# basilevh/tcow

Measured on AMD Instinct MI355X. Metric: train clips/sec (T=30, 240x320), higher is better.
Workload: dtype bf16; 1 GPU; TCOW Seeker train step: T=30 240x320 patch16, 12-layer divided space-time ViT (D=768), num_queries=3, causal_attention=1, 1 clip/GPU; clips_per_gpu=1, num_queries=3, parallelism=dp1, optimizer=AdamW lr 1e-4, clip 0.3

## Files before the change

### include/tcow_hip.h

```cpp
#ifndef TCOW_HIP_H
#define TCOW_HIP_H

#ifdef __cplusplus
extern "C" {
#endif

#define TCOW_OK 0
#define TCOW_ERR_INVALID_ARG (-1)
#define TCOW_ERR_LAUNCH (-2)
#define TCOW_ERR_UNSUPPORTED (-3)

#define TCOW_F32 0
#define TCOW_BF16 1
#define TCOW_F32X3 2

#define TCOW_ACT_NONE 0
#define TCOW_ACT_GELU 1
#define TCOW_ACT_DGELU 2
#define TCOW_ACT_GELU_DSAVE 3
#define TCOW_ACT_MUL_AUX 4

#define TCOW_ABI_VERSION 14
int tcow_version(void);
const char* tcow_last_error(void);
// ... 36 lines not shown
    float* bias_grad;
    int accumulate;
} tcow_tn_problem;
long tcow_gemm_tn_grouped_workspace_bytes(int dtype, int n, const tcow_tn_problem* problems);
int tcow_gemm_tn_grouped(void* stream, int dtype, int n, const tcow_tn_problem* problems, void* workspace, long workspace_bytes);
int tcow_gemm_tn_group_max(void);

typedef struct {
    int M, N, K;
    const float* A; long sai, sak;
    const float* B; long sbj, sbk;
    float* C; long ldc;
    int accumulate;
} tcow_sgemm;
int tcow_sgemm_x3_batched(void* stream, int n, const tcow_sgemm* problems);

int tcow_layernorm_fwd(void* stream, int dtype, int rows, int D, const float* x, long ldx, const float* gamma,
                       const float* beta, float eps, void* y, long ldy, float* mean, float* rstd);
long tcow_layernorm_bwd_workspace_bytes(int D);
int tcow_layernorm_bwd(void* stream, int dtype, int rows, int D, const void* dy, long lddy, const float* x, long ldx,
                       const float* mean, const float* rstd, const float* gamma, const float* dres, long lddres,
                       float* dx, long lddx, float* dgamma, float* dbeta, int accumulate, void* workspace,
                       long workspace_bytes, void* dx_cast, long lddx_cast, const float* cast_row_scale,
                       const float* colsum_row_scale, float* colsum_out);
typedef struct {
    const float* part; int parts, D;
    float* dgamma; float* dbeta; float* colsum_out;
    int accumulate;
} tcow_ln_fold_job;
int tcow_layernorm_bwd_parts(int rows, int with_colsum);
int tcow_layernorm_fold(void* stream, int n, const tcow_ln_fold_job* jobs);

typedef struct {
// ... 125 lines not shown
```

### tcow_amd/_lib.py

```python
import ctypes
import os

_HERE = os.path.dirname(os.path.abspath(__file__))
LIB_PATH = os.environ.get('TCOW_LIB') or os.path.join(_HERE, 'libtcow_hip.so')
LIB_PATH_FP16 = os.path.join(_HERE, 'libtcow_hip_fp16.so')

TCOW_F32, TCOW_BF16, TCOW_F32X3 = 0, 1, 2
ACT_NONE, ACT_GELU, ACT_DGELU, ACT_GELU_DSAVE, ACT_MUL_AUX = 0, 1, 2, 3, 4


class TcowError(RuntimeError):
    """Raised when a libtcow_hip entry point returns a non-zero status (message from tcow_last_error)."""


class AttnShape(ctypes.Structure):
    _fields_ = [('B', ctypes.c_int), ('T', ctypes.c_int), ('S', ctypes.c_int), ('D', ctypes.c_int),
                ('heads', ctypes.c_int), ('causal', ctypes.c_int), ('dtype', ctypes.c_int)]


class GemmArgs(ctypes.Structure):
    _fields_ = [('M', ctypes.c_int), ('N', ctypes.c_int), ('K', ctypes.c_int), ('dtype', ctypes.c_int),
                ('A', ctypes.c_void_p), ('lda', ctypes.c_long), ('W', ctypes.c_void_p), ('ldw', ctypes.c_long),
                ('C', ctypes.c_void_p), ('ldc', ctypes.c_long), ('out_f32', ctypes.c_int),
                ('bias', ctypes.c_void_p), ('row_scale', ctypes.c_void_p), ('resid', ctypes.c_void_p),
                ('ldr', ctypes.c_long), ('act', ctypes.c_int), ('aux', ctypes.c_void_p), ('ldaux', ctypes.c_long), ('tile', ctypes.c_int),
                ('bias2', ctypes.c_void_p), ('row_scale2', ctypes.c_void_p)]


class SGemm(ctypes.Structure):
    _fields_ = [('M', ctypes.c_int), ('N', ctypes.c_int), ('K', ctypes.c_int),
                ('A', ctypes.c_void_p), ('sai', ctypes.c_long), ('sak', ctypes.c_long),
                ('B', ctypes.c_void_p), ('sbj', ctypes.c_long), ('sbk', ctypes.c_long),
                ('C', ctypes.c_void_p), ('ldc', ctypes.c_long), ('accumulate', ctypes.c_int)]


class TnProblem(ctypes.Structure):
    _fields_ = [('M', ctypes.c_int), ('N', ctypes.c_int), ('K', ctypes.c_int),
                ('dY', ctypes.c_void_p), ('ldy', ctypes.c_long), ('X', ctypes.c_void_p), ('ldx', ctypes.c_long),
                ('dW', ctypes.c_void_p), ('lddw', ctypes.c_long), ('bias_grad', ctypes.c_void_p), ('accumulate', ctypes.c_int)]


class LnFoldJob(ctypes.Structure):
    _fields_ = [('part', ctypes.c_void_p), ('parts', ctypes.c_int), ('D', ctypes.c_int), ('dgamma', ctypes.c_void_p), ('dbeta', ctypes.c_void_p),
                ('colsum_out', ctypes.c_void_p), ('accumulate', ctypes.c_int)]


class MaskLossArgs(ctypes.Structure):
    _fields_ = [('n_frames', ctypes.c_long), ('frame_len', ctypes.c_long), ('frames_per_seq', ctypes.c_long),
# ... 14 lines not shown
    'tcow_version': (_i, []),
    'tcow_last_error': (ctypes.c_char_p, []),
    'tcow_gemm_nt': (_i, [_vp, ctypes.POINTER(GemmArgs)]),
    'tcow_gemm_nt_skinny_workspace_bytes': (_l, [_i, _i, _i]),
    'tcow_gemm_nt_skinny': (_i, [_vp, ctypes.POINTER(GemmArgs), _i, _vp, _l]),
    'tcow_prof_gemm_begin': (_i, [_i]),
    'tcow_prof_gemm_end': (_i, [ctypes.POINTER(ctypes.c_double), ctypes.POINTER(ctypes.c_double), ctypes.POINTER(ctypes.c_long)]),
    'tcow_prof_attn_begin': (_i, [_i]),
    'tcow_prof_attn_end': (_i, [_vp, _vp, _vp, _vp]),
    'tcow_gemm_tn_workspace_bytes': (_l, [_i, _i, _i]),
    'tcow_gemm_tn': (_i, [_vp, _i, _i, _i, _i, _vp, _l, _vp, _l, _vp, _l, _vp, _i, _vp, _l]),
    'tcow_gemm_tn_grouped_workspace_bytes': (_l, [_i, _i, _vp]),
    'tcow_gemm_tn_grouped': (_i, [_vp, _i, _i, _vp, _vp, _l]),
    'tcow_gemm_tn_group_max': (_i, []),
    'tcow_sgemm_x3_batched': (_i, [_vp, _i, _vp]),
    'tcow_layernorm_fwd': (_i, [_vp, _i, _i, _i, _vp, _l, _vp, _vp, _f, _vp, _l, _vp, _vp]),
    'tcow_layernorm_bwd_workspace_bytes': (_l, [_i]),
    'tcow_layernorm_bwd': (_i, [_vp, _i, _i, _i, _vp, _l, _vp, _l, _vp, _vp, _vp, _vp, _l, _vp, _l, _vp, _vp, _i, _vp, _l, _vp, _l, _vp, _vp, _vp]),
    'tcow_layernorm_bwd_parts': (_i, [_i, _i]),
    'tcow_layernorm_fold': (_i, [_vp, _i, _vp]),
    'tcow_attn_temporal_fwd': (_i, [_vp, _ash, _vp, _vp, _vp]),
    'tcow_attn_spatial_fwd': (_i, [_vp, _ash, _vp, _vp, _vp]),
    'tcow_attn_bwd_workspace_bytes': (_l, [_ash]),
    'tcow_attn_temporal_bwd': (_i, [_vp, _ash, _vp, _vp, _vp, _vp, _vp, _vp, _l]),
    'tcow_attn_spatial_bwd': (_i, [_vp, _ash, _vp, _vp, _vp, _vp, _vp, _vp, _l]),
    'tcow_attn_temporal_cached_fwd': (_i, [_vp, _ash, _i, _vp, _vp, _vp, _vp, _vp]),
    'tcow_cls_stream': (_i, [_vp, _i, _i, _i, _i, _vp, _vp, _vp]),
    'tcow_attn_temporal_pool_fwd': (_i, [_vp, _ash, _i, _i, _vp, _vp, _vp, _vp, _vp, _vp]),
    'tcow_cls_pool': (_i, [_vp, _i, _i, _i, _i, _vp, _vp, _i, _vp, _vp]),
    'tcow_attn_temporal_ragged_fwd': (_i, [_vp, _ash, _i, _i, _i, _vp, _vp, _vp, _vp, _vp, _vp, _vp, _vp, _vp]),
    'tcow_cls_ragged': (_i, [_vp, _i, _i, _i, _i, _vp, _vp, _i, _vp, _vp, _vp, _vp]),
# ... 76 lines not shown
```

### tcow_amd/csrc/gemm_x3.hip

```cpp
#include "gemm_f32.h"

namespace {

constexpr int XT = 128;
constexpr int XK = 32;
constexpr int XP = 80;
constexpr int XPLANE = XT * XP;

typedef __attribute__((ext_vector_type(8))) __bf16 x3_bf16x8;
typedef __attribute__((ext_vector_type(2))) __bf16 x3_bf16x2;
__device__ __forceinline__ uint32_t x3_pack(float a, float b) {
    f32x2 v = {a, b};
    return __builtin_bit_cast(uint32_t, __builtin_convertvector(v, x3_bf16x2));
}
__device__ __forceinline__ void split2(float x0, float x1, uint32_t& h, uint32_t& l) {
    h = x3_pack(x0, x1);
    l = x3_pack(x0 - __builtin_bit_cast(float, h << 16), x1 - __builtin_bit_cast(float, h & 0xffff0000u));
}

enum { LD_ANY = 0, LD_KVEC = 1, LD_RVEC = 2 };

template <int LD>
__device__ __forceinline__ void load_regs(const float* __restrict__ P, long s_row, long s_k, int row0, int nrows, int k0, int K, f32x4 (&v)[4], int tid) {
    if (LD == LD_KVEC) {
// ... 91 lines not shown
                uint32_t h, l;
                split2(v[e][2 * ps], v[e][2 * ps + 1], h, l);
                const int off = (iq + 32 * e) * XP + (kp + 8 * ps) * 4;
                *reinterpret_cast<uint32_t*>(hi_plane + off) = h;
                *reinterpret_cast<uint32_t*>(lo_plane + off) = l;
            }
    }
}

__device__ __forceinline__ int cdiv_dev(int a, int b) { return (a + b - 1) / b; }

__device__ __forceinline__ x3_bf16x8 frag(const char* plane, int row, int ks, int hi) {
    return __builtin_bit_cast(x3_bf16x8, *reinterpret_cast<const uint4*>(plane + row * XP + ks * 32 + hi * 16));
}

template <int LDA, int LDB>
__device__ __forceinline__ void gemm_x3_body(const F32Params& p, const int bid, const int kz, char* smem) {
    char* a_hi = smem; char* a_lo = smem + XPLANE; char* b_hi = smem + 2 * XPLANE; char* b_lo = smem + 3 * XPLANE;
    const int tid = threadIdx.x, lane = tid & 63, wave = tid >> 6;
    const int wm = wave >> 1, wn = wave & 1, l31 = lane & 31, hi = lane >> 5;
    const int tiles_n = cdiv_dev(p.N, XT), nblk = tiles_n * cdiv_dev(p.M, XT);
    const int q = nblk >> 3, rr = nblk & 7, xcd = bid & 7;
    const int pid = ((xcd < rr) ? xcd * (q + 1) : rr * (q + 1) + (xcd - rr) * q) + (bid >> 3);
    const int pm = pid / tiles_n;
    const int m0 = pm * XT, n0 = (pid - pm * tiles_n) * XT;
    const int kbeg = kz * p.kps;
    const int kend = (kbeg + p.kps < p.K) ? kbeg + p.kps : p.K;
    f32x16 acc[2][2];
#pragma unroll
    for (int i = 0; i < 2; ++i)
#pragma unroll
        for (int j = 0; j < 2; ++j)
// ... 24 lines not shown
                for (int j = 0; j < 2; ++j) {
                    acc[i][j] = __builtin_amdgcn_mfma_f32_32x32x16_bf16(bh[j], al[i], acc[i][j], 0, 0, 0);
                    acc[i][j] = __builtin_amdgcn_mfma_f32_32x32x16_bf16(bl[j], ah[i], acc[i][j], 0, 0, 0);
                    acc[i][j] = __builtin_amdgcn_mfma_f32_32x32x16_bf16(bh[j], ah[i], acc[i][j], 0, 0, 0);
                }
        }
        __syncthreads();
    };
    fetch(ra0, rb0, kbeg);
    __builtin_amdgcn_sched_barrier(0);
    fetch(ra1, rb1, kbeg + XK);
    __builtin_amdgcn_sched_barrier(0);
    for (int k0 = kbeg; k0 < kend; k0 += 2 * XK) {
        step(ra0, rb0, k0, k0 + 2 * XK);
        step(ra1, rb1, k0 + XK, k0 + 3 * XK);
    }
    constexpr int CT_LD = 68;
    float* ct = reinterpret_cast<float*>(smem) + wave * (32 * CT_LD);
    const int c4 = (lane & 15) * 4, r4 = lane >> 4;
    const int gn = n0 + wn * 64 + c4;
    const bool v16 = p.slab ? ((reinterpret_cast<uintptr_t>(p.slab) & 15) == 0 && (p.N & 3) == 0)
                            : (((reinterpret_cast<uintptr_t>(p.C) | reinterpret_cast<uintptr_t>(p.resid) | reinterpret_cast<uintptr_t>(p.aux) | reinterpret_cast<uintptr_t>(p.bias2)) & 15) == 0 &&
                               ((p.ldc | p.ldr | p.ldaux) & 3) == 0);
    float4 b4 = make_float4(0.f, 0.f, 0.f, 0.f);
    if (!p.slab && p.bias) {
        if (gn < p.N) b4.x = p.bias[gn];
        if (gn + 1 < p.N) b4.y = p.bias[gn + 1];
        if (gn + 2 < p.N) b4.z = p.bias[gn + 2];
        if (gn + 3 < p.N) b4.w = p.bias[gn + 3];
    }
// ... 21 lines not shown
                    if (slab) slab[(size_t)gm * p.N + gn + e] = xs[e];
                    else f32_epilogue_store(p, gm, gn + e, xs[e], bs[e]);
                }
            }
        }
    }
}

template <int LD>
__global__ __launch_bounds__(256, LD == LD_ANY ? 2 : 3) void gemm_x3_kernel(F32Params p) {
    __shared__ __attribute__((aligned(16))) char smem[4 * XPLANE];
    gemm_x3_body<LD, LD>(p, blockIdx.x, blockIdx.y, smem);
}

constexpr int X3_MAX_BATCH = 24;
struct X3Batch { F32Params p[X3_MAX_BATCH]; };
template <int LDA, int LDB>
__global__ __launch_bounds__(256, (LDA == LD_ANY || LDB == LD_ANY) ? 2 : 3) void gemm_x3_batch_kernel(X3Batch b) {
    __shared__ __attribute__((aligned(16))) char smem[4 * XPLANE];
    const F32Params& p = b.p[blockIdx.y];
    if ((int)blockIdx.x >= cdiv_dev(p.N, XT) * cdiv_dev(p.M, XT)) return;
    gemm_x3_body<LDA, LDB>(p, blockIdx.x, 0, smem);
}

}

int tcow_launch_slab_reduce(hipStream_t stream, const float* slab, int nz, long slab_stride, long rows, long cols, float* out, long ldo, int accumulate,
                            const float* bias_part, int bias_nparts, int bias_n, float* bias_out);

int tcow_gemm_nt_x3(hipStream_t stream, const tcow_gemm_args* a) {
    F32Params p;
    p.M = a->M; p.N = a->N; p.K = a->K;
    p.A = (const float*)a->A; p.sai = a->lda; p.sak = 1;
    p.B = (const float*)a->W; p.sbj = a->ldw; p.sbk = 1;
    p.C = a->C; p.ldc = a->ldc; p.bias = a->bias; p.row_scale = a->row_scale; p.resid = a->resid; p.ldr = a->ldr;
    p.act = a->act; p.aux = (float*)a->aux; p.ldaux = a->ldaux; p.bias2 = a->bias2; p.row_scale2 = a->row_scale2; p.kps = ((a->K + XK - 1) / XK) * XK; p.slab = nullptr;
    const bool vec = ((reinterpret_cast<uintptr_t>(p.A) | reinterpret_cast<uintptr_t>(p.B)) & 15) == 0 && ((p.sai | p.sbj | p.K) & 3) == 0;
// ... 27 lines not shown
    const bool vec = ((reinterpret_cast<uintptr_t>(dY) | reinterpret_cast<uintptr_t>(X)) & 15) == 0 && ((ldy | ldx | N | K) & 3) == 0;
    const dim3 grid(cdiv(K, XT) * cdiv(N, XT), nz);
    if (vec) hipLaunchKernelGGL(gemm_x3_kernel<LD_RVEC>, grid, dim3(256), 0, stream, p);
    else hipLaunchKernelGGL(gemm_x3_kernel<LD_ANY>, grid, dim3(256), 0, stream, p);
    TCOW_CHECK_LAUNCH();
    return tcow_launch_slab_reduce(stream, slab, nz, (long)N * K, N, K, dW, lddw, accumulate, bias_part, bias_nparts, N, bias_out);
}

static int x3_loader(const float* P, long s_row, long s_k, int nrows, int K) {
    const bool al = (reinterpret_cast<uintptr_t>(P) & 15) == 0;
    if (s_k == 1 && al && (s_row & 3) == 0 && (K & 3) == 0 && K >= 4) return LD_KVEC;
    if (s_row == 1 && al && (s_k & 3) == 0 && (nrows & 3) == 0 && nrows >= 4) return LD_RVEC;
    return LD_ANY;
}

extern "C" int tcow_sgemm_x3_batched(void* stream, int n, const tcow_sgemm* probs) {
    TCOW_CHECK_ARG(n >= 1 && n <= X3_MAX_BATCH && probs, "tcow_sgemm_x3_batched: 1 .. %d problems per call (got %d)", X3_MAX_BATCH, n);
    X3Batch b;
    int lda = -1, ldb = -1, maxtiles = 0;
    for (int i = 0; i < n; ++i) {
        const tcow_sgemm& s = probs[i];
        TCOW_CHECK_ARG(s.M > 0 && s.N > 0 && s.K > 0 && s.A && s.B && s.C && s.ldc >= s.N, "tcow_sgemm_x3_batched: bad problem %d", i);
        F32Params& p = b.p[i];
        p.M = s.M; p.N = s.N; p.K = s.K; p.A = s.A; p.sai = s.sai; p.sak = s.sak; p.B = s.B; p.sbj = s.sbj; p.sbk = s.sbk;
        p.C = s.C; p.ldc = s.ldc; p.bias = nullptr; p.row_scale = nullptr; p.resid = nullptr; p.ldr = 0; p.act = 0; p.aux = nullptr; p.ldaux = 0; p.bias2 = nullptr; p.row_scale2 = nullptr;
        p.kps = ((s.K + XK - 1) / XK) * XK; p.slab = nullptr;
        if (s.accumulate) { p.resid = s.C; p.ldr = s.ldc; }
        const int la = x3_loader(s.A, s.sai, s.sak, s.M, s.K), lb = x3_loader(s.B, s.sbj, s.sbk, s.N, s.K);
        lda = (lda < 0 || lda == la) ? la : LD_ANY; ldb = (ldb < 0 || ldb == lb) ? lb : LD_ANY;
        const int t = cdiv(s.N, XT) * cdiv(s.M, XT);
        if (t > maxtiles) maxtiles = t;
    }
    const dim3 grid(maxtiles, n);
    hipStream_t st = (hipStream_t)stream;
    if (lda == LD_KVEC && ldb == LD_KVEC) hipLaunchKernelGGL((gemm_x3_batch_kernel<LD_KVEC, LD_KVEC>), grid, dim3(256), 0, st, b);
    else if (lda == LD_KVEC && ldb == LD_RVEC) hipLaunchKernelGGL((gemm_x3_batch_kernel<LD_KVEC, LD_RVEC>), grid, dim3(256), 0, st, b);
    else if (lda == LD_RVEC && ldb == LD_RVEC) hipLaunchKernelGGL((gemm_x3_batch_kernel<LD_RVEC, LD_RVEC>), grid, dim3(256), 0, st, b);
    else if (lda == LD_RVEC && ldb == LD_ANY) hipLaunchKernelGGL((gemm_x3_batch_kernel<LD_RVEC, LD_ANY>), grid, dim3(256), 0, st, b);
    else hipLaunchKernelGGL((gemm_x3_batch_kernel<LD_ANY, LD_ANY>), grid, dim3(256), 0, st, b);
    TCOW_CHECK_LAUNCH();
    return TCOW_OK;
}
```

### tcow_amd/csrc/layernorm.hip

```cpp
#include <stdlib.h>

#include "common.h"

namespace {

constexpr int LN_MAXV = 8;

template <typename T, int NV, bool FULL>
__global__ __launch_bounds__(256) void ln_fwd_kernel(int rows, int D, const float* __restrict__ x, long ldx, const float* __restrict__ gamma,
                                                     const float* __restrict__ beta, float eps, T* __restrict__ y, long ldy,
                                                     float* __restrict__ mean_out, float* __restrict__ rstd_out) {
    const int lane = threadIdx.x & 63;
    const int nv = D >> 2;
    const int rstep = gridDim.x * 4;
    int row = blockIdx.x * 4 + (threadIdx.x >> 6);
    if (row >= rows) return;
    float4 g[NV], b[NV], nx[NV];
#pragma unroll
    for (int i = 0; i < NV; ++i) {
        const int c = lane + i * 64;
        if (FULL || c < nv) { g[i] = ld4(gamma + c * 4); b[i] = ld4(beta + c * 4); nx[i] = ld4(x + (size_t)row * ldx + c * 4); }
    }
    for (; row < rows; row += rstep) {
        float4 v[NV];
        float s = 0.f;
#pragma unroll
        for (int i = 0; i < NV; ++i) {
            const int c = lane + i * 64;
            if (FULL || c < nv) { v[i] = nx[i]; s += (v[i].x + v[i].y) + (v[i].z + v[i].w); }
        }
        if (row + rstep < rows) {
#pragma unroll
            for (int i = 0; i < NV; ++i) {
                const int c = lane + i * 64;
                if (FULL || c < nv) nx[i] = ld4(x + (size_t)(row + rstep) * ldx + c * 4);
            }
        }
        const float mean = wave_sum(s) / (float)D;
        float q = 0.f;
#pragma unroll
        for (int i = 0; i < NV; ++i) {
            const int c = lane + i * 64;
            if (FULL || c < nv) {
                const float a = v[i].x - mean, bb = v[i].y - mean, cc = v[i].z - mean, d = v[i].w - mean;
                q += (a * a + bb * bb) + (cc * cc + d * d);
            }
        }
        const float rstd = 1.0f / sqrtf(wave_sum(q) / (float)D + eps);
        if (lane == 0) {
            if (mean_out) mean_out[row] = mean;
// ... 120 lines not shown
        __syncthreads();
    }
}

}

int tcow_launch_row_reduce2(hipStream_t stream, const float* part, int nrows, long ld, int N1, float* out1, int N2, float* out2, int accumulate);
int tcow_launch_row_reduce_group(hipStream_t stream, int n, const float* const* part, const int* nrows, const long* ld, const int* N1, float* const* out1, const int* N2,
                                 float* const* out2, const int* N3, float* const* out3, const int* accumulate);
int tcow_launch_row_reduce3(hipStream_t stream, const float* part, int nrows, long ld, int N1, float* out1, int N2, float* out2, int N3, float* out3, int accumulate);

static const int kLnBwdBlocks = 768;
static const int kLnBwdBlocksCsum = 512;
static const int kLnFwdBlocks = 4096;

extern "C" {

int tcow_layernorm_fwd(void* stream, int dtype, int rows, int D, const float* x, long ldx, const float* gamma, const float* beta, float eps, void* y,
                       long ldy, float* mean, float* rstd) {
    TCOW_CHECK_ARG(rows > 0 && D > 0 && D % 4 == 0 && D <= 64 * 4 * LN_MAXV, "tcow_layernorm_fwd: D=%d must be a multiple of 4 and <= %d", D, 64 * 4 * LN_MAXV);
    TCOW_CHECK_ARG(x && gamma && beta && y && ldx % 4 == 0 && ldy % 4 == 0, "tcow_layernorm_fwd: bad pointers / strides");
    int fblocks = cdiv(rows, 4); if (fblocks > kLnFwdBlocks) fblocks = kLnFwdBlocks;
    const dim3 grid(fblocks), block(256);
    if (dtype != TCOW_BF16 && dtype != TCOW_F32) { tcow_set_error("tcow_layernorm_fwd: unknown dtype %d", dtype); return TCOW_ERR_INVALID_ARG; }
    const int nvl = (D / 4 + 63) / 64;
#define LN_FWD(NVV, FULLV)                                                                                                                               \
    do {                                                                                                                                          \
        if (dtype == TCOW_BF16) hipLaunchKernelGGL((ln_fwd_kernel<bf16_t, NVV, FULLV>), grid, block, 0, (hipStream_t)stream, rows, D, x, ldx, gamma, beta, eps, (bf16_t*)y, ldy, mean, rstd); \
        else hipLaunchKernelGGL((ln_fwd_kernel<float, NVV, FULLV>), grid, block, 0, (hipStream_t)stream, rows, D, x, ldx, gamma, beta, eps, (float*)y, ldy, mean, rstd); \
    } while (0)
    const bool full = D == 256 * nvl && nvl <= 4;
    if (full) { if (nvl == 1) LN_FWD(1, true); else if (nvl == 2) LN_FWD(2, true); else if (nvl == 3) LN_FWD(3, true); else LN_FWD(4, true); }
    else if (nvl <= 1) LN_FWD(1, false); else if (nvl == 2) LN_FWD(2, false); else if (nvl == 3) LN_FWD(3, false); else if (nvl == 4) LN_FWD(4, false); else LN_FWD(8, false);
#undef LN_FWD
    TCOW_CHECK_LAUNCH();
    return TCOW_OK;
}

long tcow_layernorm_bwd_workspace_bytes(int D) { return (long)kLnBwdBlocks * 3 * D * 4; }

int tcow_layernorm_bwd(void* stream, int dtype, int rows, int D, const void* dy, long lddy, const float* x, long ldx, const float* mean,
                       const float* rstd, const float* gamma, const float* dres, long lddres, float* dx, long lddx, float* dgamma, float* dbeta,
                       int accumulate, void* workspace, long workspace_bytes, void* dx_cast, long lddx_cast, const float* cast_row_scale,
                       const float* colsum_row_scale, float* colsum_out) {
    TCOW_CHECK_ARG(rows > 0 && D > 0 && D % 4 == 0 && D <= 64 * 4 * LN_MAXV, "tcow_layernorm_bwd: bad D=%d", D);
    TCOW_CHECK_ARG(dy && x && mean && rstd && gamma && dx, "tcow_layernorm_bwd: null pointer");
    TCOW_CHECK_ARG(!dx_cast || lddx_cast % 4 == 0, "tcow_layernorm_bwd: dx_cast stride must be a multiple of 4");
    const bool want_param_grads = dgamma != nullptr || dbeta != nullptr;
    TCOW_CHECK_ARG(!want_param_grads || (dgamma && dbeta && workspace && workspace_bytes >= tcow_layernorm_bwd_workspace_bytes(D)),
                   "tcow_layernorm_bwd: parameter gradients need dgamma, dbeta and a workspace of %ld bytes", tcow_layernorm_bwd_workspace_bytes(D));
    TCOW_CHECK_ARG(!colsum_out || want_param_grads, "tcow_layernorm_bwd: colsum_out rides on the parameter-gradient pass (dgamma / dbeta needed)");
// ... 46 lines not shown
```

### tcow_amd/engine.py

```python
import os
import torch

from . import ops
from .ops import ACT_GELU, ACT_GELU_DSAVE, ACT_MUL_AUX
from .operands import fold_on


def _layout(module):
    if module.attention_type == 'divided_space_time':
        return 20, dict(tn=0, tqkv=2, tproj=4, tfc=6, n1=8, qkv=10, proj=12, n2=14, fc1=16, fc2=18)
    return 12, dict(n1=0, qkv=2, proj=4, n2=6, fc1=8, fc2=10)


def _joint_rows(module, g, dev):
    def build():
        B, T, S = g['B'], g['T'], g['S']
        r = torch.arange(B * T * S, device=dev).reshape(B, T * S)
        keep = torch.ones(T * S, dtype=torch.bool, device=dev)
        keep[torch.arange(1, T, device=dev) * S] = False
        return r[:, keep].reshape(-1).contiguous()
    return module._operands.constant(('jrows', g['B'], str(dev)), build)


def group_sizes(depth, spec=None):
# ... 165 lines not shown
    joint = module.attention_type != 'divided_space_time'
    fold = fold_on(module)
    amode = gmode if gmode == ops.F32X3 else mode
    shape_attn = ops.attn_shape(amode, B, T, S, D, heads, ca)
    if joint:
        jrows = _joint_rows(module, g, dev)
        Lj = 1 + T * (S - 1)
        shape_joint = ops.attn_shape(amode, B, 1, Lj, D, heads, 0)
    for i in range(module.network_depth):
        q = params[5 + i * BP: 5 + (i + 1) * BP]
        P_ = lambda name, k=0: q[ix[name] + k].detach()
        n1_w, n1_b, qkv_b, proj_b, n2_w, n2_b, fc1_w, fc1_b, fc2_b = P_('n1'), P_('n1', 1), P_('qkv', 1), P_('proj', 1), P_('n2'), P_('n2', 1), P_('fc1'), P_('fc1', 1), P_('fc2', 1)
        dp = dps[i]
        st = {}
        R0 = X
        if joint:
            V = E(M, D); mu1 = E(M, dtype=f32) if save else None; rs1 = E(M, dtype=f32) if save else None
            ops.layernorm_fwd(mode, R0, n1_w, n1_b, V, mu1, rs1)
            QKV2 = E(M, 3 * D)
            ops.gemm_nt(gmode, V, W(q[ix['qkv']]), QKV2, bias=qkv_b, **sk)
            QJ = QKV2.index_select(0, jrows)
            OJ = E(B * Lj, D); lse_s = E(B * Lj, heads, dtype=f32) if save else None
            ops.attn_fwd(shape_joint, True, QJ, OJ, lse_s)
            O2 = torch.zeros(M, D, dtype=dt, device=dev)
            O2.index_copy_(0, jrows, OJ)
            rs_s = dp['s']
            R2 = E(M, D, dtype=f32) if save else R0
            ops.gemm_nt(gmode, O2, W(q[ix['proj']]), R2, bias=proj_b, row_scale=rs_s, resid=R0, **sk)
            if save:
                st.update(R1=R0, mu1=mu1, rs1=rs1, V=V, QKV_s=QJ, O_s=O2, OJ=OJ, lse_s=lse_s, rs_s=rs_s)
# ... 21 lines not shown
                st.update(R0=R0, mu0=mu0, rs0=rs0, U=U, QKV_t=QKV, O_t=O, lse_t=lse_t, Pj=Pj)
            V = E(M, D); mu1 = E(M, dtype=f32) if save else None; rs1 = E(M, dtype=f32) if save else None
            ops.layernorm_fwd(mode, R1, n1_w, n1_b, V, mu1, rs1)
            QKV2 = E(M, 3 * D)
            ops.gemm_nt(gmode, V, W(q[ix['qkv']]), QKV2, bias=qkv_b, **sk)
            O2 = E(M, D); lse_s = E(M, heads, dtype=f32) if save else None
            ops.attn_fwd(shape_attn, True, QKV2, O2, lse_s)
            rs_s = dp['s']
            if not use_cls:
                rs_s = mask0 if rs_s is None else rs_s * mask0
            R2 = E(M, D, dtype=f32) if save else R1
            ops.gemm_nt(gmode, O2, W(q[ix['proj']]), R2, bias=proj_b, row_scale=rs_s, resid=R1, **sk)
            if use_cls and stream is not None:
                stream.cls_row(i, R2, B, T, S)
            elif use_cls:
                ops.cls_merge(R2, B, T, S, 1 if ca == 1 else 0)
            if save:
                st.update(R1=R1, mu1=mu1, rs1=rs1, V=V, QKV_s=QKV2, O_s=O2, lse_s=lse_s, rs_s=rs_s)
        Wn = E(M, D); mu2 = E(M, dtype=f32) if save else None; rs2 = E(M, dtype=f32) if save else None
        ops.layernorm_fwd(mode, R2, n2_w, n2_b, Wn, mu2, rs2)
        Hd = fc1_w.shape[0]
        pre = E(M, Hd) if save else None
        H = E(M, Hd)
        ops.gemm_nt(gmode, Wn, W(q[ix['fc1']]), H, bias=fc1_b, act=ACT_GELU_DSAVE if save else ACT_GELU, aux=pre, **sk)
        R3 = E(M, D, dtype=f32) if save else R2
        ops.gemm_nt(gmode, H, W(q[ix['fc2']]), R3, bias=fc2_b, row_scale=dp['m'], resid=R2, **sk)
        if save:
            st.update(R2=R2, mu2=mu2, rs2=rs2, Wn=Wn, pre=pre, H=H)
            sv['blocks'].append(st)
        X = R3

    nb = 5 + module.network_depth * BP
    norm_w, norm_b, head_w, head_b = params[nb], params[nb + 1], params[nb + 2], params[nb + 3]
    feat32 = X
    if module.norm_embeddings:
# ... 137 lines not shown
    late = set()
    if fold:
        for j in range(depth):
            late.update((5 + j * BP + ix['tproj'], 5 + j * BP + ix['tproj'] + 1, 5 + j * BP + ix['tfc']))
    late_flat = bucket(sorted(late)) if late else None
    blk_idx = lambda lo_, hi_: [j for j in range(5 + lo_ * BP, 5 + hi_ * BP) if j not in late]
    flat_cur = bucket((list(range(0, 5)) if top_lo == 0 else []) + blk_idx(top_lo, depth) + head_idx)
    fold_jobs = []

    def fold_tmp(i):
        return opnd.buffer(('foldtmp', i, str(dev)), lambda: (torch.empty(D, D, dtype=f32, device=dev), torch.empty(D, dtype=f32, device=dev)))

    def finish_fold_group():
        if not fold_jobs:
            return
        nt_, r1_, tn_, gv_ = [], [], [], []
        for (i, tW, tb) in fold_jobs:
            o_ = 5 + i * BP
            wfc, wp, bp = params[o_ + ix['tfc']].detach(), params[o_ + ix['tproj']].detach(), params[o_ + ix['tproj'] + 1].detach()
            nt_.append((tW, wp.t(), grads[o_ + ix['tfc']]))
            r1_.append((tb.view(-1, 1), bp.view(1, -1), grads[o_ + ix['tfc']]))
            tn_.append((wfc.t(), tW, grads[o_ + ix['tproj']]))
            gv_.append((wfc.t(), tb.view(-1, 1), grads[o_ + ix['tproj'] + 1].view(-1, 1)))
        for c0 in range(0, len(nt_), 24):
            ops.sgemm_batched(nt_[c0:c0 + 24]); ops.sgemm_batched(r1_[c0:c0 + 24], accumulate=True)
            ops.sgemm_batched(tn_[c0:c0 + 24]); ops.sgemm_batched(gv_[c0:c0 + 24])
        fold_jobs.clear()

    if d_mask is None:
        d_mask = torch.zeros(B, Co, T, module.frame_height, module.frame_width, dtype=f32, device=dev)
    d_mask = d_mask.to(f32).contiguous()
    dpooled = E(B * T, Co, sv['h'], sv['w'], dtype=f32)
    mask_amax = None
    if ls_mode == 'dynamic' and sv['bilinear'] and sv['stp'] == 4 and sv['h'] > 4 and sv['w'] > 4:
        _, mask_amax = ops.upsample_bwd_amax(d_mask, B, T, Co, sv['h'], sv['w'], sv['stp'], dpooled)
    else:
        if ls_mode == 'dynamic' and d_mask.numel():
            mask_amax = d_mask.abs().amax()
        ops.upsample_bwd(d_mask, B, T, Co, sv['h'], sv['w'], sv['stp'], sv['bilinear'], dpooled)
    gscale, inv_gscale = choose_scale(mask_amax)
    if gscale is not None:
# ... 183 lines not shown
```

### tcow_amd/ops.py

```python
import ctypes
import threading

import numpy as np
import torch

from . import _lib as L

F32, BF16 = L.TCOW_F32, L.TCOW_BF16
F32X3 = L.TCOW_F32X3
ACT_NONE, ACT_GELU, ACT_DGELU, ACT_GELU_DSAVE, ACT_MUL_AUX = L.ACT_NONE, L.ACT_GELU, L.ACT_DGELU, L.ACT_GELU_DSAVE, L.ACT_MUL_AUX


FP16 = 16


def tdtype(mode):
    return torch.bfloat16 if mode == BF16 else torch.float16 if mode == FP16 else torch.float32


def is16(mode):
    return mode in (BF16, FP16)


def _sel(mode):
# ... 125 lines not shown
    return int(L.lib().tcow_gemm_tn_group_max())


def gemm_tn_grouped(mode, problems):
    n = len(problems)
    arr = (L.TnProblem * n)()
    for i, (dY, X, dW, db, *acc) in enumerate(problems):
        _need_cuda(dY, X, dW)
        arr[i] = L.TnProblem(dY.shape[0], dY.shape[1], X.shape[1], dY.data_ptr(), dY.stride(0), X.data_ptr(), X.stride(0), dW.data_ptr(), dW.stride(0), _p(db),
                             int(acc[0]) if acc else 0)
    lib, dm = _sel(mode)
    ws = workspace(lib.tcow_gemm_tn_grouped_workspace_bytes(dm, n, arr), problems[0][0].device, 'tn')
    L.check(lib.tcow_gemm_tn_grouped(_stream(), dm, n, arr, ws.data_ptr(), ws.numel()), 'tcow_gemm_tn_grouped', lib)


def sgemm_batched(problems, accumulate=False):
    n = len(problems)
    arr = (L.SGemm * n)()
    for i, (A, B, C) in enumerate(problems):
        _need_cuda(A, B, C)
        M, K = A.shape
        N = B.shape[1]
        assert B.shape[0] == K and C.shape == (M, N) and C.stride(1) == 1 and A.dtype == B.dtype == C.dtype == torch.float32
        arr[i] = L.SGemm(M, N, K, A.data_ptr(), A.stride(0), A.stride(1), B.data_ptr(), B.stride(1), B.stride(0), C.data_ptr(), C.stride(0), 1 if accumulate else 0)
    L.check(L.lib().tcow_sgemm_x3_batched(_stream(), n, arr), 'tcow_sgemm_x3_batched')


def layernorm_fwd(mode, x, gamma, beta, out, mean=None, rstd=None, eps=1e-6):
    rows, D = x.shape
    lib, dm = _sel(mode)
    L.check(lib.tcow_layernorm_fwd(_stream(), dm, rows, D, x.data_ptr(), x.stride(0), gamma.data_ptr(), beta.data_ptr(), eps,
                                       out.data_ptr(), out.stride(0), _p(mean), _p(rstd)), 'tcow_layernorm_fwd', lib)
    return out


def layernorm_bwd(mode, dy, x, mean, rstd, gamma, dres, dx, dgamma=None, dbeta=None, accumulate=False, dx_cast=None, cast_scale=None,
                  colsum_out=None, colsum_scale=None, defer=None):
    rows, D = x.shape
    lib, dm = _sel(mode)
    if defer is not None and dgamma is not None:
        ws = workspace(lib.tcow_layernorm_bwd_workspace_bytes(D), x.device, 'ln_defer%d' % len(defer))
        defer.append((lib, ws, int(lib.tcow_layernorm_bwd_parts(rows, 1 if colsum_out is not None else 0)), D, dgamma, dbeta, colsum_out, bool(accumulate)))
        accumulate = int(accumulate) | 2
    else:
        ws = workspace(lib.tcow_layernorm_bwd_workspace_bytes(D), x.device, 'ln')
# ... 383 lines not shown
```

Baseline: 37.48 clips/s.

## Fuse rank-1 and column riders into batched x3 sgemm; fold CLS merge into LayerNorm

The batched fp32 x3 GEMM kernel now takes optional riders. A rank-1 outer-product term is added into the tile accumulators with extra MFMAs, and a column matrix-vector product runs in extra grid blocks. This lets the temporal fold group issue two batched launches instead of four. Separately, the CLS-token merge before the second LayerNorm is fused into the LayerNorm forward kernel for the causal case: each row reads its CLS source and writes the merged row back. This removes a separate merge launch and a pass over the residual, at the cost of more template variants and more complex indexing.

```diff
diff --git a/include/tcow_hip.h b/include/tcow_hip.h
--- a/include/tcow_hip.h
+++ b/include/tcow_hip.h
@@ -74,9 +74,21 @@
     int accumulate;
 } tcow_sgemm;
 int tcow_sgemm_x3_batched(void* stream, int n, const tcow_sgemm* problems);
+typedef struct {
+    int M, N, K;
+    const float* A; long sai, sak;
+    const float* B; long sbj, sbk;
+    float* C; long ldc;
+    int accumulate;
+    const float* col_b; float* col_c;
+    const float* r1_u; const float* r1_v;
+} tcow_sgemm_rider;
+int tcow_sgemm_x3_riders(void* stream, int n, const tcow_sgemm_rider* problems);
 
 int tcow_layernorm_fwd(void* stream, int dtype, int rows, int D, const float* x, long ldx, const float* gamma,
                        const float* beta, float eps, void* y, long ldy, float* mean, float* rstd);
+int tcow_layernorm_fwd_cls(void* stream, int dtype, int B, int T, int S, int D, float* x, long ldx, const float* gamma,
+                           const float* beta, float eps, void* y, long ldy, float* mean, float* rstd, int how);
 long tcow_layernorm_bwd_workspace_bytes(int D);
 int tcow_layernorm_bwd(void* stream, int dtype, int rows, int D, const void* dy, long lddy, const float* x, long ldx,
                        const float* mean, const float* rstd, const float* gamma, const float* dres, long lddres,
diff --git a/tcow_amd/_lib.py b/tcow_amd/_lib.py
--- a/tcow_amd/_lib.py
+++ b/tcow_amd/_lib.py
@@ -32,6 +32,10 @@
                 ('A', ctypes.c_void_p), ('sai', ctypes.c_long), ('sak', ctypes.c_long),
                 ('B', ctypes.c_void_p), ('sbj', ctypes.c_long), ('sbk', ctypes.c_long),
                 ('C', ctypes.c_void_p), ('ldc', ctypes.c_long), ('accumulate', ctypes.c_int)]
+
+
+class SGemmRider(ctypes.Structure):
+    _fields_ = SGemm._fields_ + [('col_b', ctypes.c_void_p), ('col_c', ctypes.c_void_p), ('r1_u', ctypes.c_void_p), ('r1_v', ctypes.c_void_p)]
 
 
 class TnProblem(ctypes.Structure):
@@ -76,7 +80,9 @@
     'tcow_gemm_tn_grouped': (_i, [_vp, _i, _i, _vp, _vp, _l]),
     'tcow_gemm_tn_group_max': (_i, []),
     'tcow_sgemm_x3_batched': (_i, [_vp, _i, _vp]),
+    'tcow_sgemm_x3_riders': (_i, [_vp, _i, _vp]),
     'tcow_layernorm_fwd': (_i, [_vp, _i, _i, _i, _vp, _l, _vp, _vp, _f, _vp, _l, _vp, _vp]),
+    'tcow_layernorm_fwd_cls': (_i, [_vp, _i, _i, _i, _i, _i, _vp, _l, _vp, _vp, _f, _vp, _l, _vp, _vp, _i]),
     'tcow_layernorm_bwd_workspace_bytes': (_l, [_i]),
     'tcow_layernorm_bwd': (_i, [_vp, _i, _i, _i, _vp, _l, _vp, _l, _vp, _vp, _vp, _vp, _l, _vp, _l, _vp, _vp, _i, _vp, _l, _vp, _l, _vp, _vp, _vp]),
     'tcow_layernorm_bwd_parts': (_i, [_i, _i]),
diff --git a/tcow_amd/csrc/gemm_x3.hip b/tcow_amd/csrc/gemm_x3.hip
--- a/tcow_amd/csrc/gemm_x3.hip
+++ b/tcow_amd/csrc/gemm_x3.hip
@@ -129,8 +129,17 @@
     return __builtin_bit_cast(x3_bf16x8, *reinterpret_cast<const uint4*>(plane + row * XP + ks * 32 + hi * 16));
 }
 
-template <int LDA, int LDB>
-__device__ __forceinline__ void gemm_x3_body(const F32Params& p, const int bid, const int kz, char* smem) {
+struct X3Prob {
+    int M, N, K, accumulate;
+    const float* A; long sai, sak;
+    const float* B; long sbj, sbk;
+    float* C; long ldc;
+    const float* col_b; float* col_c;
+    const float* r1_u; const float* r1_v;
+};
+
+template <int LDA, int LDB, bool RID = false>
+__device__ __forceinline__ void gemm_x3_body(const F32Params& p, const int bid, const int kz, char* smem, const X3Prob* rd = nullptr) {
     char* a_hi = smem; char* a_lo = smem + XPLANE; char* b_hi = smem + 2 * XPLANE; char* b_lo = smem + 3 * XPLANE;
     const int tid = threadIdx.x, lane = tid & 63, wave = tid >> 6;
     const int wm = wave >> 1, wn = wave & 1, l31 = lane & 31, hi = lane >> 5;
@@ -185,6 +194,34 @@
     for (int k0 = kbeg; k0 < kend; k0 += 2 * XK) {
         step(ra0, rb0, k0, k0 + 2 * XK);
         step(ra1, rb1, k0 + XK, k0 + 3 * XK);
+    }
+    if constexpr (RID) {
+        if (rd->r1_u) {
+            x3_bf16x8 ah[2], al[2], bh[2], bl[2];
+#pragma unroll
+            for (int i = 0; i < 2; ++i) {
+                const int gm = m0 + wm * 64 + i * 32 + l31, gnn = n0 + wn * 64 + i * 32 + l31;
+                const float u = (hi == 0 && gm < p.M) ? rd->r1_u[gm] : 0.f, v = (hi == 0 && gnn < p.N) ? rd->r1_v[gnn] : 0.f;
+                uint32_t h, l;
+                split2(u, 0.f, h, l);
+                ah[i] = __builtin_bit_cast(x3_bf16x8, make_uint4(h, 0u, 0u, 0u)); al[i] = __builtin_bit_cast(x3_bf16x8, make_uint4(l, 0u, 0u, 0u));
+                split2(v, 0.f, h, l);
+                bh[i] = __builtin_bit_cast(x3_bf16x8, make_uint4(h, 0u, 0u, 0u)); bl[i] = __builtin_bit_cast(x3_bf16x8, make_uint4(l, 0u, 0u, 0u));
+            }
+#pragma unroll
+            for (int i = 0; i < 2; ++i)
+#pragma unroll
+                for (int j = 0; j < 2; ++j) {
+                    f32x16 r;
+#pragma unroll
+                    for (int e = 0; e < 16; ++e) r[e] = 0.f;
+                    r = __builtin_amdgcn_mfma_f32_32x32x16_bf16(bh[j], al[i], r, 0, 0, 0);
+                    r = __builtin_amdgcn_mfma_f32_32x32x16_bf16(bl[j], ah[i], r, 0, 0, 0);
+                    r = __builtin_amdgcn_mfma_f32_32x32x16_bf16(bh[j], ah[i], r, 0, 0, 0);
+#pragma unroll
+                    for (int e = 0; e < 16; ++e) acc[i][j][e] += r[e];
+                }
+        }
     }
     constexpr int CT_LD = 68;
     float* ct = reinterpret_cast<float*>(smem) + wave * (32 * CT_LD);
@@ -236,13 +273,30 @@
 }
 
 constexpr int X3_MAX_BATCH = 24;
-struct X3Batch { F32Params p[X3_MAX_BATCH]; };
-template <int LDA, int LDB>
-__global__ __launch_bounds__(256, (LDA == LD_ANY || LDB == LD_ANY) ? 2 : 3) void gemm_x3_batch_kernel(X3Batch b) {
+struct X3Batch { X3Prob p[X3_MAX_BATCH]; int maxtiles; };
+
+__device__ __forceinline__ void x3_plain_params(F32Params& p, const X3Prob& q) {
+    p.M = q.M; p.N = q.N; p.K = q.K; p.A = q.A; p.sai = q.sai; p.sak = q.sak; p.B = q.B; p.sbj = q.sbj; p.sbk = q.sbk;
+    p.C = q.C; p.ldc = q.ldc; p.bias = nullptr; p.row_scale = nullptr; p.resid = q.accumulate ? q.C : nullptr; p.ldr = q.ldc; p.act = 0; p.aux = nullptr; p.ldaux = 0;
+    p.bias2 = nullptr; p.row_scale2 = nullptr; p.kps = ((q.K + XK - 1) / XK) * XK; p.slab = nullptr;
+}
+
+template <int LDA, int LDB, int LDV>
+__global__ __launch_bounds__(256, (LDA == LD_ANY || LDB == LD_ANY || LDV == LD_ANY) ? 2 : 3) void gemm_x3_batch_kernel(X3Batch b) {
     __shared__ __attribute__((aligned(16))) char smem[4 * XPLANE];
-    const F32Params& p = b.p[blockIdx.y];
-    if ((int)blockIdx.x >= cdiv_dev(p.N, XT) * cdiv_dev(p.M, XT)) return;
-    gemm_x3_body<LDA, LDB>(p, blockIdx.x, 0, smem);
+    const X3Prob& q = b.p[blockIdx.y];
+    const int bx = blockIdx.x;
+    F32Params p;
+    x3_plain_params(p, q);
+    if (bx >= b.maxtiles) {
+        const int t = bx - b.maxtiles;
+        if (!q.col_b || t >= cdiv_dev(q.M, XT)) return;
+        p.N = 1; p.B = q.col_b; p.sbj = 0; p.sbk = 1; p.C = q.col_c; p.ldc = 1; p.resid = q.accumulate ? q.col_c : nullptr; p.ldr = 1;
+        gemm_x3_body<LDA, LDV>(p, t, 0, smem);
+        return;
+    }
+    if (!q.C || bx >= cdiv_dev(q.N, XT) * cdiv_dev(q.M, XT)) return;
+    gemm_x3_body<LDA, LDB, true>(p, bx, 0, smem, &q);
 }
 
 }
@@ -300,30 +354,67 @@
     return LD_ANY;
 }
 
+static int x3_launch_batch(hipStream_t st, int n, X3Batch& b) {
+    int lda = -1, ldb = -1, ldv = -1, maxtiles = 0, maxcol = 0;
+    for (int i = 0; i < n; ++i) {
+        const X3Prob& q = b.p[i];
+        if (q.C) {
+            const int la = x3_loader(q.A, q.sai, q.sak, q.M, q.K), lb = x3_loader(q.B, q.sbj, q.sbk, q.N, q.K);
+            lda = (lda < 0 || lda == la) ? la : LD_ANY; ldb = (ldb < 0 || ldb == lb) ? lb : LD_ANY;
+        }
+        if (q.col_b) {
+            const int la = x3_loader(q.A, q.sai, q.sak, q.M, q.K), lv = x3_loader(q.col_b, 0, 1, 1, q.K);
+            lda = (lda < 0 || lda == la) ? la : LD_ANY; ldv = (ldv < 0 || ldv == lv) ? lv : LD_ANY;
+        }
+        const int t = q.C ? cdiv(q.N, XT) * cdiv(q.M, XT) : 0, ct = q.col_b ? cdiv(q.M, XT) : 0;
+        if (t > maxtiles) maxtiles = t;
+        if (ct > maxcol) maxcol = ct;
+    }
+    b.maxtiles = maxtiles;
+    const dim3 grid(maxtiles + maxcol, n);
+    if (ldb < 0) ldb = lda;
+    const bool vk = ldv < 0 || ldv == LD_KVEC;
+    if (lda == LD_KVEC && ldb == LD_KVEC && vk) hipLaunchKernelGGL((gemm_x3_batch_kernel<LD_KVEC, LD_KVEC, LD_KVEC>), grid, dim3(256), 0, st, b);
+    else if (lda == LD_KVEC && ldb == LD_RVEC && vk) hipLaunchKernelGGL((gemm_x3_batch_kernel<LD_KVEC, LD_RVEC, LD_KVEC>), grid, dim3(256), 0, st, b);
+    else if (lda == LD_RVEC && ldb == LD_RVEC && vk) hipLaunchKernelGGL((gemm_x3_batch_kernel<LD_RVEC, LD_RVEC, LD_KVEC>), grid, dim3(256), 0, st, b);
+    else if (lda == LD_RVEC && ldb == LD_ANY) hipLaunchKernelGGL((gemm_x3_batch_kernel<LD_RVEC, LD_ANY, LD_ANY>), grid, dim3(256), 0, st, b);
+    else hipLaunchKernelGGL((gemm_x3_batch_kernel<LD_ANY, LD_ANY, LD_ANY>), grid, dim3(256), 0, st, b);
+    TCOW_CHECK_LAUNCH();
+    return TCOW_OK;
+}
+
 extern "C" int tcow_sgemm_x3_batched(void* stream, int n, const tcow_sgemm* probs) {
     TCOW_CHECK_ARG(n >= 1 && n <= X3_MAX_BATCH && probs, "tcow_sgemm_x3_batched: 1 .. %d problems per call (got %d)", X3_MAX_BATCH, n);
     X3Batch b;
-    int lda = -1, ldb = -1, maxtiles = 0;
     for (int i = 0; i < n; ++i) {
         const tcow_sgemm& s = probs[i];
         TCOW_CHECK_ARG(s.M > 0 && s.N > 0 && s.K > 0 && s.A && s.B && s.C && s.ldc >= s.N, "tcow_sgemm_x3_batched: bad problem %d", i);
-        F32Params& p = b.p[i];
-        p.M = s.M; p.N = s.N; p.K = s.K; p.A = s.A; p.sai = s.sai; p.sak = s.sak; p.B = s.B; p.sbj = s.sbj; p.sbk = s.sbk;
-        p.C = s.C; p.ldc = s.ldc; p.bias = nullptr; p.row_scale = nullptr; p.resid = nullptr; p.ldr = 0; p.act = 0; p.aux = nullptr; p.ldaux = 0; p.bias2 = nullptr; p.row_scale2 = nullptr;
-        p.kps = ((s.K + XK - 1) / XK) * XK; p.slab = nullptr;
-        if (s.accumulate) { p.resid = s.C; p.ldr = s.ldc; }
-        const int la = x3_loader(s.A, s.sai, s.sak, s.M, s.K), lb = x3_loader(s.B, s.sbj, s.sbk, s.N, s.K);
-        lda = (lda < 0 || lda == la) ? la : LD_ANY; ldb = (ldb < 0 || ldb == lb) ? lb : LD_ANY;
-        const int t = cdiv(s.N, XT) * cdiv(s.M, XT);
-        if (t > maxtiles) maxtiles = t;
-    }
-    const dim3 grid(maxtiles, n);
-    hipStream_t st = (hipStream_t)stream;
-    if (lda == LD_KVEC && ldb == LD_KVEC) hipLaunchKernelGGL((gemm_x3_batch_kernel<LD_KVEC, LD_KVEC>), grid, dim3(256), 0, st, b);
-    else if (lda == LD_KVEC && ldb == LD_RVEC) hipLaunchKernelGGL((gemm_x3_batch_kernel<LD_KVEC, LD_RVEC>), grid, dim3(256), 0, st, b);
-    else if (lda == LD_RVEC && ldb == LD_RVEC) hipLaunchKernelGGL((gemm_x3_batch_kernel<LD_RVEC, LD_RVEC>), grid, dim3(256), 0, st, b);
-    else if (lda == LD_RVEC && ldb == LD_ANY) hipLaunchKernelGGL((gemm_x3_batch_kernel<LD_RVEC, LD_ANY>), grid, dim3(256), 0, st, b);
-    else hipLaunchKernelGGL((gemm_x3_batch_kernel<LD_ANY, LD_ANY>), grid, dim3(256), 0, st, b);
-    TCOW_CHECK_LAUNCH();
-    return TCOW_OK;
-}
+        X3Prob& q = b.p[i];
+        q.M = s.M; q.N = s.N; q.K = s.K; q.accumulate = s.accumulate != 0; q.A = s.A; q.sai = s.sai; q.sak = s.sak; q.B = s.B; q.sbj = s.sbj; q.sbk = s.sbk;
+        q.C = s.C; q.ldc = s.ldc; q.col_b = nullptr; q.col_c = nullptr; q.r1_u = nullptr; q.r1_v = nullptr;
+    }
+    return x3_launch_batch((hipStream_t)stream, n, b);
+}
+
+extern "C" int tcow_sgemm_x3_riders(void* stream, int n, const tcow_sgemm_rider* probs) {
+    TCOW_CHECK_ARG(n >= 1 && n <= X3_MAX_BATCH && probs, "tcow_sgemm_x3_riders: 1 .. %d problems per call (got %d)", X3_MAX_BATCH, n);
+    static_assert(sizeof(X3Batch) <= 4096, "the problem records travel as kernel arguments");
+    X3Batch b;
+    for (int i = 0; i < n; ++i) {
+        const tcow_sgemm_rider& s = probs[i];
+        const bool mat = s.B != nullptr, r1 = s.r1_u != nullptr, col = s.col_b != nullptr, tile = mat || r1;
+        TCOW_CHECK_ARG((mat || r1 || col) && s.M > 0, "tcow_sgemm_x3_riders: problem %d has no product, no rank-1 term and no column rider (or M <= 0)", i);
+        TCOW_CHECK_ARG(!tile || (s.C && s.N > 0 && s.ldc >= s.N), "tcow_sgemm_x3_riders: problem %d: C [M,N] with ldc >= N is needed", i);
+        TCOW_CHECK_ARG(!(mat || col) || (s.A && s.K > 0), "tcow_sgemm_x3_riders: problem %d: A [M,K] is needed", i);
+        TCOW_CHECK_ARG(!r1 || s.r1_v, "tcow_sgemm_x3_riders: problem %d: the rank-1 term needs u and v", i);
+        TCOW_CHECK_ARG(!col || s.col_c, "tcow_sgemm_x3_riders: problem %d: the column rider needs col_b and col_c", i);
+        TCOW_CHECK_ARG(mat || !(r1 && col), "tcow_sgemm_x3_riders: problem %d: a column rider beside a rank-1 term needs the matrix product too", i);
+        X3Prob& q = b.p[i];
+        q.M = s.M; q.N = tile ? s.N : 0; q.K = s.K; q.accumulate = s.accumulate != 0; q.A = s.A; q.sai = s.sai; q.sak = s.sak; q.B = s.B; q.sbj = s.sbj; q.sbk = s.sbk;
+        q.C = tile ? s.C : nullptr; q.ldc = s.ldc; q.col_b = s.col_b; q.col_c = col ? s.col_c : nullptr; q.r1_u = s.r1_u; q.r1_v = s.r1_v;
+        if (r1 && !mat) {
+            q.K = 1; q.A = s.r1_u; q.sai = 1; q.sak = 1; q.B = s.r1_v; q.sbj = 1; q.sbk = 1; q.r1_u = nullptr; q.r1_v = nullptr;
+        }
+    }
+    return x3_launch_batch((hipStream_t)stream, n, b);
+}
diff --git a/tcow_amd/csrc/layernorm.hip b/tcow_amd/csrc/layernorm.hip
--- a/tcow_amd/csrc/layernorm.hip
+++ b/tcow_amd/csrc/layernorm.hip
@@ -6,20 +6,24 @@
 
 constexpr int LN_MAXV = 8;
 
-template <typename T, int NV, bool FULL>
+template <typename T, int NV, bool FULL, bool CLS = false>
 __global__ __launch_bounds__(256) void ln_fwd_kernel(int rows, int D, const float* __restrict__ x, long ldx, const float* __restrict__ gamma,
                                                      const float* __restrict__ beta, float eps, T* __restrict__ y, long ldy,
-                                                     float* __restrict__ mean_out, float* __restrict__ rstd_out) {
+                                                     float* __restrict__ mean_out, float* __restrict__ rstd_out, float* xw = nullptr, int S = 1, int TS = 1) {
     const int lane = threadIdx.x & 63;
     const int nv = D >> 2;
     const int rstep = gridDim.x * 4;
     int row = blockIdx.x * 4 + (threadIdx.x >> 6);
     if (row >= rows) return;
+    auto src = [&](int r) { if (!CLS) return r; const int u = __builtin_amdgcn_readfirstlane(r); return u % S == 0 ? u - u % TS : u; };
     float4 g[NV], b[NV], nx[NV];
-#pragma unroll
-    for (int i = 0; i < NV; ++i) {
-        const int c = lane + i * 64;
-        if (FULL || c < nv) { g[i] = ld4(gamma + c * 4); b[i] = ld4(beta + c * 4); nx[i] = ld4(x + (size_t)row * ldx + c * 4); }
+    {
+        const int sr = src(row);
+#pragma unroll
+        for (int i = 0; i < NV; ++i) {
+            const int c = lane + i * 64;
+            if (FULL || c < nv) { g[i] = ld4(gamma + c * 4); b[i] = ld4(beta + c * 4); nx[i] = ld4(x + (size_t)sr * ldx + c * 4); }
+        }
     }
     for (; row < rows; row += rstep) {
         float4 v[NV];
@@ -30,10 +34,18 @@
             if (FULL || c < nv) { v[i] = nx[i]; s += (v[i].x + v[i].y) + (v[i].z + v[i].w); }
         }
         if (row + rstep < rows) {
-#pragma unroll
-            for (int i = 0; i < NV; ++i) {
-                const int c = lane + i * 64;
-                if (FULL || c < nv) nx[i] = ld4(x + (size_t)(row + rstep) * ldx + c * 4);
+            const int sr = src(row + rstep);
+#pragma unroll
+            for (int i = 0; i < NV; ++i) {
+                const int c = lane + i * 64;
+                if (FULL || c < nv) nx[i] = ld4(x + (size_t)sr * ldx + c * 4);
+            }
+        }
+        if (CLS && src(row) != row) {
+#pragma unroll
+            for (int i = 0; i < NV; ++i) {
+                const int c = lane + i * 64;
+                if (FULL || c < nv) st4(xw + (size_t)row * ldx + c * 4, v[i]);
             }
         }
         const float mean = wave_sum(s) / (float)D;
@@ -184,10 +196,9 @@
 static const int kLnBwdBlocksCsum = 512;
 static const int kLnFwdBlocks = 4096;
 
-extern "C" {
-
-int tcow_layernorm_fwd(void* stream, int dtype, int rows, int D, const float* x, long ldx, const float* gamma, const float* beta, float eps, void* y,
-                       long ldy, float* mean, float* rstd) {
+template <bool CLS>
+static int ln_fwd_launch(void* stream, int dtype, int rows, int D, const float* x, long ldx, const float* gamma, const float* beta, float eps, void* y,
+                         long ldy, float* mean, float* rstd, float* xw, int S, int TS) {
     TCOW_CHECK_ARG(rows > 0 && D > 0 && D % 4 == 0 && D <= 64 * 4 * LN_MAXV, "tcow_layernorm_fwd: D=%d must be a multiple of 4 and <= %d", D, 64 * 4 * LN_MAXV);
     TCOW_CHECK_ARG(x && gamma && beta && y && ldx % 4 == 0 && ldy % 4 == 0, "tcow_layernorm_fwd: bad pointers / strides");
     int fblocks = cdiv(rows, 4); if (fblocks > kLnFwdBlocks) fblocks = kLnFwdBlocks;
@@ -196,8 +207,8 @@
     const int nvl = (D / 4 + 63) / 64;
 #define LN_FWD(NVV, FULLV)                                                                                                                               \
     do {                                                                                                                                          \
-        if (dtype == TCOW_BF16) hipLaunchKernelGGL((ln_fwd_kernel<bf16_t, NVV, FULLV>), grid, block, 0, (hipStream_t)stream, rows, D, x, ldx, gamma, beta, eps, (bf16_t*)y, ldy, mean, rstd); \
-        else hipLaunchKernelGGL((ln_fwd_kernel<float, NVV, FULLV>), grid, block, 0, (hipStream_t)stream, rows, D, x, ldx, gamma, beta, eps, (float*)y, ldy, mean, rstd); \
+        if (dtype == TCOW_BF16) hipLaunchKernelGGL((ln_fwd_kernel<bf16_t, NVV, FULLV, CLS>), grid, block, 0, (hipStream_t)stream, rows, D, x, ldx, gamma, beta, eps, (bf16_t*)y, ldy, mean, rstd, xw, S, TS); \
+        else hipLaunchKernelGGL((ln_fwd_kernel<float, NVV, FULLV, CLS>), grid, block, 0, (hipStream_t)stream, rows, D, x, ldx, gamma, beta, eps, (float*)y, ldy, mean, rstd, xw, S, TS); \
     } while (0)
     const bool full = D == 256 * nvl && nvl <= 4;
     if (full) { if (nvl == 1) LN_FWD(1, true); else if (nvl == 2) LN_FWD(2, true); else if (nvl == 3) LN_FWD(3, true); else LN_FWD(4, true); }
@@ -205,6 +216,24 @@
 #undef LN_FWD
     TCOW_CHECK_LAUNCH();
     return TCOW_OK;
+}
+
+extern "C" {
+
+int tcow_layernorm_fwd(void* stream, int dtype, int rows, int D, const float* x, long ldx, const float* gamma, const float* beta, float eps, void* y,
+                       long ldy, float* mean, float* rstd) {
+    return ln_fwd_launch<false>(stream, dtype, rows, D, x, ldx, gamma, beta, eps, y, ldy, mean, rstd, nullptr, 1, 1);
+}
+
+int tcow_layernorm_fwd_cls(void* stream, int dtype, int B, int T_, int S, int D, float* x, long ldx, const float* gamma, const float* beta, float eps, void* y,
+                           long ldy, float* mean, float* rstd, int how) {
+    TCOW_CHECK_ARG(B > 0 && T_ > 0 && S > 1 && (long)B * T_ * S < (1L << 31) && (how == 0 || how == 1), "tcow_layernorm_fwd_cls: bad geometry B=%d T=%d S=%d how=%d", B, T_, S, how);
+    const int rows = B * T_ * S;
+    if (how == 1) return ln_fwd_launch<true>(stream, dtype, rows, D, x, ldx, gamma, beta, eps, y, ldy, mean, rstd, x, S, T_ * S);
+    TCOW_CHECK_ARG(ldx == D, "tcow_layernorm_fwd_cls: how = 0 needs a contiguous x (ldx == D)");
+    const int e = tcow_cls_merge(stream, B, T_, S, D, x, 0, 0);
+    if (e != TCOW_OK) return e;
+    return ln_fwd_launch<false>(stream, dtype, rows, D, x, ldx, gamma, beta, eps, y, ldy, mean, rstd, nullptr, 1, 1);
 }
 
 long tcow_layernorm_bwd_workspace_bytes(int D) { return (long)kLnBwdBlocks * 3 * D * 4; }
diff --git a/tcow_amd/engine.py b/tcow_amd/engine.py
--- a/tcow_amd/engine.py
+++ b/tcow_amd/engine.py
@@ -203,6 +203,7 @@
         dp = dps[i]
         st = {}
         R0 = X
+        cls_rule = None
         if joint:
             V = E(M, D); mu1 = E(M, dtype=f32) if save else None; rs1 = E(M, dtype=f32) if save else None
             ops.layernorm_fwd(mode, R0, n1_w, n1_b, V, mu1, rs1)
@@ -254,11 +255,11 @@
             if use_cls and stream is not None:
                 stream.cls_row(i, R2, B, T, S)
             elif use_cls:
-                ops.cls_merge(R2, B, T, S, 1 if ca == 1 else 0)
+                cls_rule = (B, T, S, 1 if ca == 1 else 0)
             if save:
                 st.update(R1=R1, mu1=mu1, rs1=rs1, V=V, QKV_s=QKV2, O_s=O2, lse_s=lse_s, rs_s=rs_s)
         Wn = E(M, D); mu2 = E(M, dtype=f32) if save else None; rs2 = E(M, dtype=f32) if save else None
-        ops.layernorm_fwd(mode, R2, n2_w, n2_b, Wn, mu2, rs2)
+        ops.layernorm_fwd(mode, R2, n2_w, n2_b, Wn, mu2, rs2, cls=cls_rule)
         Hd = fc1_w.shape[0]
         pre = E(M, Hd) if save else None
         H = E(M, Hd)
@@ -426,17 +427,14 @@
     def finish_fold_group():
         if not fold_jobs:
             return
-        nt_, r1_, tn_, gv_ = [], [], [], []
+        nt_, tn_ = [], []
         for (i, tW, tb) in fold_jobs:
             o_ = 5 + i * BP
             wfc, wp, bp = params[o_ + ix['tfc']].detach(), params[o_ + ix['tproj']].detach(), params[o_ + ix['tproj'] + 1].detach()
-            nt_.append((tW, wp.t(), grads[o_ + ix['tfc']]))
-            r1_.append((tb.view(-1, 1), bp.view(1, -1), grads[o_ + ix['tfc']]))
-            tn_.append((wfc.t(), tW, grads[o_ + ix['tproj']]))
-            gv_.append((wfc.t(), tb.view(-1, 1), grads[o_ + ix['tproj'] + 1].view(-1, 1)))
+            nt_.append(ops.Rider(tW, wp.t(), grads[o_ + ix['tfc']], r1=(tb, bp)))
+            tn_.append(ops.Rider(wfc.t(), tW, grads[o_ + ix['tproj']], col=(tb, grads[o_ + ix['tproj'] + 1])))
         for c0 in range(0, len(nt_), 24):
-            ops.sgemm_batched(nt_[c0:c0 + 24]); ops.sgemm_batched(r1_[c0:c0 + 24], accumulate=True)
-            ops.sgemm_batched(tn_[c0:c0 + 24]); ops.sgemm_batched(gv_[c0:c0 + 24])
+            ops.sgemm_batched(nt_[c0:c0 + 24]); ops.sgemm_batched(tn_[c0:c0 + 24])
         fold_jobs.clear()
 
     if d_mask is None:
diff --git a/tcow_amd/ops.py b/tcow_amd/ops.py
--- a/tcow_amd/ops.py
+++ b/tcow_amd/ops.py
@@ -163,7 +163,39 @@
     L.check(lib.tcow_gemm_tn_grouped(_stream(), dm, n, arr, ws.data_ptr(), ws.numel()), 'tcow_gemm_tn_grouped', lib)
 
 
+class Rider(tuple):
+
+    def __new__(cls, A, B, C, col=None, r1=None):
+        self = super().__new__(cls, (A, B, C))
+        self.col, self.r1 = col, r1
+        return self
+
+
+def _sgemm_riders(problems, accumulate):
+    n = len(problems)
+    arr = (L.SGemmRider * n)()
+    for i, pr in enumerate(problems):
+        A, B, C = pr
+        col, r1 = getattr(pr, 'col', None), getattr(pr, 'r1', None)
+        vecs = [t for pair in (col, r1) if pair is not None for t in pair]
+        _need_cuda(*[t for t in (A, B, C) if t is not None], *vecs)
+        assert all(t.dtype == torch.float32 for t in (A, B, C) if t is not None) and all(t.dtype == torch.float32 and t.is_contiguous() and t.dim() == 1 for t in vecs)
+        M = A.shape[0] if A is not None else C.shape[0]
+        K = A.shape[1] if A is not None else 0
+        N = C.shape[1] if C is not None else 0
+        assert C is None or (C.shape[0] == M and C.stride(1) == 1)
+        assert B is None or (A is not None and C is not None and B.shape == (K, N))
+        assert col is None or (A is not None and col[0].numel() == K and col[1].numel() == M)
+        assert r1 is None or (C is not None and r1[0].numel() == M and r1[1].numel() == N)
+        arr[i] = L.SGemmRider(M, N, K, _p(A), A.stride(0) if A is not None else 0, A.stride(1) if A is not None else 0,
+                              _p(B), B.stride(1) if B is not None else 0, B.stride(0) if B is not None else 0, _p(C), C.stride(0) if C is not None else 0,
+                              1 if accumulate else 0, _p(col[0]) if col else None, _p(col[1]) if col else None, _p(r1[0]) if r1 else None, _p(r1[1]) if r1 else None)
+    L.check(L.lib().tcow_sgemm_x3_riders(_stream(), n, arr), 'tcow_sgemm_x3_riders')
+
+
 def sgemm_batched(problems, accumulate=False):
+    if any(isinstance(pr, Rider) for pr in problems):
+        return _sgemm_riders(problems, accumulate)
     n = len(problems)
     arr = (L.SGemm * n)()
     for i, (A, B, C) in enumerate(problems):
@@ -175,9 +207,15 @@
     L.check(L.lib().tcow_sgemm_x3_batched(_stream(), n, arr), 'tcow_sgemm_x3_batched')
 
 
-def layernorm_fwd(mode, x, gamma, beta, out, mean=None, rstd=None, eps=1e-6):
+def layernorm_fwd(mode, x, gamma, beta, out, mean=None, rstd=None, eps=1e-6, cls=None):
     rows, D = x.shape
     lib, dm = _sel(mode)
+    if cls is not None:
+        B, T, S, how = cls
+        assert rows == B * T * S
+        L.check(lib.tcow_layernorm_fwd_cls(_stream(), dm, B, T, S, D, x.data_ptr(), x.stride(0), gamma.data_ptr(), beta.data_ptr(), eps,
+                                           out.data_ptr(), out.stride(0), _p(mean), _p(rstd), int(how)), 'tcow_layernorm_fwd_cls', lib)
+        return out
     L.check(lib.tcow_layernorm_fwd(_stream(), dm, rows, D, x.data_ptr(), x.stride(0), gamma.data_ptr(), beta.data_ptr(), eps,
                                        out.data_ptr(), out.stride(0), _p(mean), _p(rstd)), 'tcow_layernorm_fwd', lib)
     return out
```

After: 37.63 clips/s, median of 6. About the same (+0.4%).
